# guenthermi/postgres-word2vec

Measured on AMD Instinct MI355X. Metric: batched IVFADC kNN queries/sec (k=5) + recall@5, 3Mx300d, higher is better.
Workload: dtype f32; 1 GPU; IVFADC batch (ivfadc_batch_search generalised to nprobe), 3000000x300d, C=1000, m=12, K=1024, nprobe=10, k=5, batch=1024 queries per GPU, replicated index, queries sharded by rank; N=3000000, d=300, C=1000, m=12, K=1024, nprobe=10, k=5, batch_per_gpu=1024, parallelism=dp1, world_size=1, backend=none (single GPU), batches_in_flight=4

## Files before the change

postgres-word2vec_amd/csrc/fused5.h:

```cpp
#pragma once
#include <hip/hip_runtime.h>
#include <stdint.h>

#include "refine.h"
#include "coarse.h"
#include "scan_tail5.h"

namespace freddy {

static constexpr int SCAN5_G = 16;
static constexpr int SCAN5_PROF_WGS = 1024;

__host__ __device__ __forceinline__ constexpr int filt5_bias(int p, int m) { return FILT5_VMAX + (p < 32768 - FILT5_VMAX * m ? 1 : 0); }
__device__ __forceinline__ uint32_t lane_byte4() {
  uint32_t x;
  asm volatile("v_mbcnt_lo_u32_b32 %0, -1, 0\n\tv_mbcnt_hi_u32_b32 %0, -1, %0\n\tv_lshlrev_b32 %0, 2, %0" : "=v"(x));
  return x;
}
typedef short s2v __attribute__((ext_vector_type(2)));
__device__ __forceinline__ uint32_t pk_add_i16(uint32_t x, uint32_t y) {
  return __builtin_bit_cast(uint32_t, __builtin_bit_cast(s2v, x) + __builtin_bit_cast(s2v, y));
}

template <int S, int QT>
__device__ __forceinline__ void query_codebook5_body(const float* __restrict__ queries, const float* __restrict__ cbT,
                                                     const float* __restrict__ cmax, float* __restrict__ qn,
                                                     float* __restrict__ qscale, uint32_t* __restrict__ qc,
                                                     int Q, int d, int m, int K, int bx, int by, unsigned char* smem,
                                                     uint32_t* __restrict__ qc8 = nullptr) {
  static_assert(QT == 16, "one 16-lane group per query");
  constexpr int SP = (S + 3) & ~3;
  float (*qs)[SP] = reinterpret_cast<float (*)[SP]>(smem);
  float* inv_s = reinterpret_cast<float*>(smem + QT * SP * 4);
  const int tid = threadIdx.x, p = bx, q0 = by * QT;
  static_assert(S <= 32 && SP % 4 == 0, "one k-step of v_mfma_f32_16x16x32_f16 covers a position");
  ch8v bh[8], bl[8];
  auto load_b = [&](int g) {
    const ch8v* src = reinterpret_cast<const ch8v*>(cbT) + ((size_t)p * 8 + g) * (CBF_GROUP_HALVES / 8) + (tid & 63);
#pragma unroll
    for (int t = 0; t < 8; ++t) { bh[t] = src[(size_t)t * 128]; bl[t] = src[(size_t)t * 128 + 64]; }
  };
  load_b((tid >> 6) * 2);
  const int ecb = reinterpret_cast<const int*>(cbT)[cbf_exp_offset(m) + p];
  for (int i = tid; i < QT * SP; i += 256) {
    const int qi = i / SP, j = i - qi * SP;
    qs[qi][j] = (j < S && q0 + qi < Q) ? queries[(size_t)(q0 + qi) * d + p * S + j] : 0.0f;
  }
  {
    const int qi = tid >> 4, pp = tid & 15, q = q0 + qi;
    float best = 0.0f;
    if (pp < m && q < Q) {
      float n2 = 0.0f;
      for (int j = 0; j < S; ++j) { const float v = queries[(size_t)q * d + pp * S + j]; n2 = __builtin_fmaf(v, v, n2); }
      const float nrm = __builtin_sqrtf(n2) * (1.0f + 1e-5f);
      if (p == 0) qn[(size_t)q * m + pp] = nrm;
      best = 2.0f * nrm * cmax[pp];
    }
#pragma unroll
    for (int o = 8; o > 0; o >>= 1) best = fmaxf(best, __shfl_xor(best, o, 64));
    if (pp == 0) {
      const float sc = q < Q ? best * (1.0f / (float)FILT5_VMAX) * (1.0f + 1e-6f) : 0.0f;
      inv_s[qi] = (sc > 0.0f && sc < 1e30f) ? 1.0f / sc : 0.0f;
      if (p == 0 && q < Q) qscale[q] = sc;
    }
  }
  {
    typedef float f4v __attribute__((ext_vector_type(4)));
    __syncthreads();
    const int wave = tid >> 6, lane = tid & 63, col = lane & 15, kq = lane >> 4;
    const int nq = (Q - q0 < QT) ? Q - q0 : QT;
    ch8v ah, al;
    int eq = 0;
    {
      f4v x0 = f4v{0.0f, 0.0f, 0.0f, 0.0f}, x1 = x0;
      if (8 * kq < SP) x0 = *reinterpret_cast<const f4v*>(&qs[col][8 * kq]);
      if (8 * kq + 4 < SP) x1 = *reinterpret_cast<const f4v*>(&qs[col][8 * kq + 4]);
      const float x[8] = {x0.x, x0.y, x0.z, x0.w, x1.x, x1.y, x1.z, x1.w};
      float am = 0.0f;
#pragma unroll
      for (int j = 0; j < 8; ++j) am = fmaxf(am, __builtin_fabsf(x[j]));
      am = fmaxf(am, __shfl_xor(am, 16, 64));
      am = fmaxf(am, __shfl_xor(am, 32, 64));
      if (am > 0.0f && am < 3e38f) { (void)__builtin_frexpf(am, &eq); eq = CBF_EXP - eq; }
#pragma unroll
      for (int j = 0; j < 8; ++j) {
        const float v = __builtin_ldexpf(x[j], eq);
        const _Float16 hh = (_Float16)v;
        ah[j] = hh;
        al[j] = (_Float16)(v - (float)hh);
      }
    }
    int unscale[4];
#pragma unroll
    for (int reg = 0; reg < 4; ++reg) unscale[reg] = -(__shfl(eq, 4 * kq + reg, 64) + ecb);
    const float vmax = (float)FILT5_VMAX;
    const int bias = filt5_bias(p, m);
#pragma unroll
    for (int gg = 0; gg < 2; ++gg) {
      const int g = wave * 2 + gg;
      f4v acc[4][2];
#pragma unroll
      for (int i = 0; i < 4; ++i)
#pragma unroll
        for (int e = 0; e < 2; ++e) acc[i][e] = __builtin_amdgcn_mfma_f32_16x16x32_f16(al, bh[2 * i + e], f4v{0.0f, 0.0f, 0.0f, 0.0f}, 0, 0, 0);
#pragma unroll
      for (int i = 0; i < 4; ++i)
#pragma unroll
        for (int e = 0; e < 2; ++e) acc[i][e] = __builtin_amdgcn_mfma_f32_16x16x32_f16(ah, bl[2 * i + e], acc[i][e], 0, 0, 0);
#pragma unroll
      for (int i = 0; i < 4; ++i)
#pragma unroll
        for (int e = 0; e < 2; ++e) acc[i][e] = __builtin_amdgcn_mfma_f32_16x16x32_f16(ah, bh[2 * i + e], acc[i][e], 0, 0, 0);
      if (gg == 0) load_b(g + 1);
#pragma unroll
      for (int reg = 0; reg < 4; ++reg) {
        const int qi = 4 * kq + reg;
        if (qi < nq) {
          const float inv = inv_s[qi];
          uint32_t wd[4];
#pragma unroll
          for (int i = 0; i < 4; ++i) {
            const int i0 = (int)fminf(fmaxf(__builtin_rintf(-2.0f * __builtin_ldexpf(acc[i][0][reg], unscale[reg]) * inv), -vmax), vmax) + bias;
            const int i1 = (int)fminf(fmaxf(__builtin_rintf(-2.0f * __builtin_ldexpf(acc[i][1][reg], unscale[reg]) * inv), -vmax), vmax) + bias;
            wd[i] = (uint32_t)i0 | ((uint32_t)i1 << 16);
          }
          *reinterpret_cast<uint4*>(qc + ((size_t)(q0 + qi) * m + p) * 512 + 4 * (16 * g + col)) = uint4{wd[0], wd[1], wd[2], wd[3]};
          if (qc8) qc8[((size_t)(q0 + qi) * m + p) * 128 + (16 * g + col)] = (wd[0] & 0xffffu) | (wd[1] << 16);
        }
      }
    }
  }
}
#define FREDDY_TABLE_UNIT_KERNEL __global__ __launch_bounds__(256) __attribute__((amdgpu_waves_per_eu(4)))
template <int S, int QT>
static constexpr int query_codebook5_lds() { return QT * ((S + 3) & ~3) * 4 + QT * 4; }
template <int S, int QT>
FREDDY_TABLE_UNIT_KERNEL void query_codebook5_kernel(const float* __restrict__ queries, const float* __restrict__ cbT,
                                                             const float* __restrict__ cmax, float* __restrict__ qn,
                                                             float* __restrict__ qscale, uint32_t* __restrict__ qc,
                                                             int Q, int d, int m, int K, uint32_t* __restrict__ qc8) {
  __shared__ __attribute__((aligned(16))) unsigned char smem[query_codebook5_lds<S, QT>()];
  query_codebook5_body<S, QT>(queries, cbT, cmax, qn, qscale, qc, Q, d, m, K, blockIdx.x, blockIdx.y, smem, qc8);
}

struct CoarseTableArgs {
  const float* queries;
  const float* coarseF; const float* cn2; float* dist; float* qn2; int Q, Cpad, d, dp; ZeroArgs z; int coarse_gx, coarse_gy;
  const float* cbT; const float* cmax; float* qn; float* qscale; uint32_t* qc; int m, K;
  float* tmin; int C;
  const ch8v* coarseH; int ec;
  uint32_t* qc8;
};
template <int S, int QT, bool H16 = false>
FREDDY_TABLE_UNIT_KERNEL void coarse_table5_kernel(CoarseTableArgs a) {
  extern __shared__ __attribute__((aligned(16))) unsigned char smem[];
  const int n_coarse = a.coarse_gx * a.coarse_gy;
  const int b = blockIdx.x;
  if (b < n_coarse) {
    if constexpr (H16)
      coarse_approx16_body(a.queries, a.coarseH, a.ec, a.cn2, a.dist, a.qn2, a.Q, a.Cpad, a.d, a.z, b % a.coarse_gx, b / a.coarse_gx,
                           a.coarse_gx, a.coarse_gy, smem, a.tmin, a.C);
    else
    coarse_approx_body(a.queries, a.coarseF, a.cn2, a.dist, a.qn2, a.Q, a.Cpad, a.d, a.dp, a.z, b % a.coarse_gx, b / a.coarse_gx,
                       a.coarse_gx, a.coarse_gy, smem, a.tmin, a.C);
  } else {
    const int t = b - n_coarse;
    query_codebook5_body<S, QT>(a.queries, a.cbT, a.cmax, a.qn, a.qscale, a.qc, a.Q, a.d, a.m, a.K, t % a.m, t / a.m, smem, a.qc8);
  }
}

template <int M>
__global__ __launch_bounds__(256) void entry_record5_kernel(RecordArgs a) {
  const int lane = threadIdx.x & 63;
  const int e = blockIdx.x * 4 + (threadIdx.x >> 6);
  if (a.elastic && blockIdx.x == 0 && threadIdx.x == 0) __hip_atomic_fetch_add(a.elastic + EL_PENDING, a.n_announce, FREDDY_RLX_AGENT);
  if (e >= a.n_groups[0]) return;
  const int cell = a.group_cell[e], first = a.group_first[e], gc = a.group_cnt[e];
  const int cnt = gc & 0xff, chunk = gc >> 8;
  int32_t* rec = a.records + (size_t)e * REC_DW;
  if (lane == 0) {
    const int b0 = a.blk_off[cell] + chunk * FUSED_UNIT_BLOCKS;
    int nb = a.blk_off[cell + 1] - b0;
    if (nb > FUSED_UNIT_BLOCKS) nb = FUSED_UNIT_BLOCKS;
    int rows = a.list_off[cell + 1] - a.list_off[cell] - chunk * (FUSED_UNIT_BLOCKS * 64);
    if (rows > FUSED_UNIT_BLOCKS * 64) rows = FUSED_UNIT_BLOCKS * 64;
    rec[0] = cell; rec[1] = cnt; rec[2] = chunk; rec[3] = b0; rec[4] = nb; rec[5] = rows;
  }
  if (lane < 16) {
    const int it = lane < cnt ? a.sorted_item[first + lane] : -1;
    const int q = a.item_query[it >= 0 ? it : a.sorted_item[first]];
    const float sc = a.qscale[q];
    ItemBounds ib = item_bounds(0.0f, 0.0f, a.sentinel);
    if (it >= 0) ib = item_bounds(a.item_dist[it], filter_width5<M>(a.qn + (size_t)q * M, a.pmax, sc), a.sentinel);
    rec[8 + lane] = it;
    rec[24 + lane] = q;
    rec[40 + lane] = (int32_t)__float_as_uint(ib.off);
    rec[56 + lane] = (int32_t)__float_as_uint(ib.e);
    rec[72 + lane] = (int32_t)__float_as_uint(ib.shift);
    rec[88 + lane] = (int32_t)ib.lo_bits;
    rec[104 + lane] = (int32_t)ib.hi_bits;
    rec[128 + lane] = (int32_t)__float_as_uint((it >= 0 && sc < 1e30f) ? sc : 0.0f);
    const float A = it >= 0 ? a.item_dist[it] : -1.0f;
    const bool fin = it >= 0 && ib.e < 1e30f && A >= 0.0f && A < 1e30f;
    rec[144 + lane] = (int32_t)__float_as_uint(fin ? A * (1.0f + 2e-5f) : __uint_as_float(0x7f800000u));
    rec[160 + lane] = (int32_t)__float_as_uint(fin ? A * (1.0f - 2e-5f) : 0.0f);
  }
}

template <int M, bool FULLK, bool CAND, bool PROF, bool U8, bool ELASTIC>
__device__ __forceinline__ void ivf_filter5_body(const FilterArgs& a) {
  static_assert(!(U8 && FULLK), "one byte per code: K <= 256");
  constexpr int G = SCAN5_G, RMAX = FUSED_RMAX, NG = SPEC2_NG;
  constexpr int NP = M / 2;
  constexpr int ROWB = G * 2;
  constexpr int HROWB = 16;
  static_assert(M == 12 && G == 16 && SPEC2_NB == 8, "layout");
  typedef uint32_t u2 __attribute__((ext_vector_type(2)));
  typedef uint32_t u4 __attribute__((ext_vector_type(4)));
  extern __shared__ __attribute__((aligned(16))) unsigned char smem[];
  unsigned char* slab = smem;
  uint32_t* colmin = reinterpret_cast<uint32_t*>(smem + a.desc_offset);
  uint32_t* thr_s = colmin + 16 * 64;
  int32_t* dsc = reinterpret_cast<int32_t*>(smem + a.desc_offset + 4096 + 64);
  int32_t* gidq = dsc + 2 * REC_DW;
  float* rt_s = reinterpret_cast<float*>(gidq + 4);

  const int tid = threadIdx.x, lane = tid & 63;
  const int wave = __builtin_amdgcn_readfirstlane(tid >> 6);
  const bool builder = wave < SPEC2_NB;
  const int K = FULLK ? 1024 : a.K;
  const uint32_t HALFB = (uint32_t)K * HROWB;
  const uint32_t POSB = 2u * HALFB;
  const uint32_t BUFB = 2u * POSB;
  const int n_work = a.n_groups[0];

  int cur = 0, ei = 0;
  const int n_own = ELASTIC ? a.n_own : (int)gridDim.x;
  const bool extra = ELASTIC && (int)blockIdx.x >= n_own;
  if (!extra) {
    if (tid == 0) {
      gidq[0] = (int)blockIdx.x; gidq[1] = n_own + atomicAdd(a.work_counter, 1);
      if constexpr (ELASTIC) {
        __hip_atomic_fetch_sub(a.elastic + EL_PENDING, 1, FREDDY_RLX_AGENT);
        if ((int)blockIdx.x < n_work) __hip_atomic_fetch_add(a.elastic + EL_ACTIVE, 1, FREDDY_RLX_AGENT);
      }
    }
    if (tid < REC_DW) dsc[tid] = a.records[(size_t)blockIdx.x * REC_DW + tid];
  } else if (tid == 0) {
    const int pend = __hip_atomic_load(a.elastic + EL_PENDING, FREDDY_RLX_AGENT);
    const int claims = __hip_atomic_load(a.work_counter, FREDDY_RLX_AGENT);
// ... 341 lines not shown
```

postgres-word2vec_amd/csrc/ivfadc.hip:

```cpp
#include "internal.h"

#include <functional>

#include "kernels.h"
#include "scan_common.h"
#include "fused3.h"
#include "fused5.h"
#include "fused8.h"
#include "one.h"
#include "sparse5.h"
#include "coarse.h"
#include "multi.h"
#include "io_kernels.h"
#include "bigk.h"
#include "ivf_host.h"
#include "query_ids.h"

static void (*scan_kernel(bool m12, int V, bool floor))(ScanArgs) {
  void (*k)(ScanArgs) = nullptr;
  if (floor) return V != 16 ? nullptr : m12 ? &adc_scan_kernel<12, 16, true> : &adc_scan_kernel<0, 16, true>;
  with_V(V, [&](auto v) { k = m12 ? &adc_scan_kernel<12, decltype(v)::value> : &adc_scan_kernel<0, decltype(v)::value>; });
  return k;
}
static void (*filter_kernel(bool whole, bool u8, bool k1024, bool counts_rows, bool prof, bool elastic = false))(FilterArgs) {
// ... 61 lines not shown
  const int passes = (2 * k + BIGK_PASS - 1) / BIGK_PASS;
  const int nsel = passes * BIGK_PASS;
  int npad = 2048;
  while (npad < k + nsel) npad *= 2;
  if (ws->w_bigsel.ensure(sizeof(u64) * (size_t)ma.n_active * nsel) || ws->w_floor.ensure(sizeof(u64) * (size_t)std::max(Q, 1)))
    return fail(FREDDY_E_NOMEM, "workspace allocation failed (k=%d)", k);
  SelectArgs se;
  se.part = sa.part; se.active = ma.active; se.sel = ws->w_bigsel.as<u64>(); se.floor = ws->w_floor.as<u64>();
  se.parts_per_query = ma.parts_per_query; se.nsel = nsel;
  int32_t* const cand_count = sa.cand_count;
  for (int p = 0; p < passes; ++p) {
    sa.floor = p ? ws->w_floor.as<u64>() : nullptr;
    sa.cand_count = p ? nullptr : cand_count;
    if (int rc = launch_scan(ix, s, sa, n_items)) return rc;
    se.pass = p;
    timed_launch(ix, s, "merge_select", [&] { hipLaunchKernelGGL(merge_select_kernel, dim3(ma.n_active), dim3(64), 0, s, se); });
    HIP_TRY(hipGetLastError());
  }
  BigkArgs b;
  b.sel = se.sel; b.active = ma.active; b.pos_to_id = ma.pos_to_id; b.round_rows = ma.round_rows; b.cand_count = ma.cand_count;
  b.out_ids = ma.out_ids; b.out_dist = ma.out_dist; b.found = ma.found; b.next_active = ma.next_active; b.n_next = ma.n_next;
  b.status = ma.status; b.n_active = ma.n_active; b.nsel = nsel; b.npad = npad; b.k = k; b.found_rule = ma.found_rule;
  b.first_round = ma.first_round; b.sentinel = ma.sentinel;
  timed_launch(ix, s, "bigk_replay", [&] {
    hipLaunchKernelGGL(bigk_replay_kernel, dim3(ma.n_active), dim3(BIGK_T), bigk_lds_bytes(npad, k), s, b);
  });
  HIP_TRY(hipGetLastError());
  return 0;
}

int launch_lut(freddy_gpu_index* ix, hipStream_t s, const float* vecs, const int32_t* item_cell,
                      float* lut, int n_items, const float* coarse, const int32_t* item_query) {
  if (n_items <= 0) return 0;
  int ipw = (int)std::max<int64_t>(1, ((int64_t)ix->m * n_items + 4095) / 4096);
  ipw = std::min(ipw, 64);
  dim3 grid((unsigned)ix->m, (unsigned)((n_items + ipw - 1) / ipw));
  const int m = ix->m, K = ix->K, d = ix->d, S = ix->S;
  timed_launch(ix, s, "lut_build", [&] {
    if (S == 25) hipLaunchKernelGGL((lut_build_kernel<25, 4>), grid, dim3(WG), 0, s, vecs, item_cell, ix->cbT, lut, n_items, ipw, m, K, d, coarse, item_query);
    else if (S == 10) hipLaunchKernelGGL((lut_build_kernel<10, 4>), grid, dim3(WG), 0, s, vecs, item_cell, ix->cbT, lut, n_items, ipw, m, K, d, coarse, item_query);
    else if (S == 20) hipLaunchKernelGGL((lut_build_kernel<20, 4>), grid, dim3(WG), 0, s, vecs, item_cell, ix->cbT, lut, n_items, ipw, m, K, d, coarse, item_query);
    else hipLaunchKernelGGL(lut_build_generic_kernel, grid, dim3(WG), 0, s, vecs, item_cell, ix->cbT, lut, n_items, ipw, m, K, d, S, coarse, item_query);
  });
  HIP_TRY(hipGetLastError());
  return 0;
}


static bool ivf_coarse_by_pieces(const IvfRun& r) { return r.approx && r.fused && r.scan_kernel == 5; }
static int ivf_coarse(IvfRun& r, int q_lo = 0, int q_n = -1) {
  Workspace* ws = r.ws;
  freddy_gpu_index* ix = r.ix;
  hipStream_t s = r.s;
  const int Q = r.Q, d = ix->d, C = ix->C, m = ix->m, K = ix->K, Cpad = ix->Cpad;
  if (q_n < 0) { q_lo = 0; q_n = Q; }
  if ((q_lo != 0 || q_n != Q) && !ivf_coarse_by_pieces(r)) return fail(FREDDY_E_ARG, "internal: this path launches its coarse kernel once");
  const int used_words = (C + 31) / 32;
  const bool small_zero = !r.tiled && d <= 1024;
  if (!r.tiled && !small_zero) {
    HIP_TRY(hipMemsetAsync(ws->w_used.p, 0, sizeof(uint32_t) * (size_t)Q * used_words, s));
    HIP_TRY(hipMemsetAsync(ws->w_cnt.p, 0, sizeof(int32_t) * 8, s));
  }
  ZeroArgs za;
  za.p[0] = ws->w_used.as<uint32_t>(); za.n[0] = Q * used_words;
  za.p[1] = ws->w_cnt.as<uint32_t>(); za.n[1] = 8;
  za.p[2] = r.fused ? ws->w_cellcnt.as<uint32_t>() : nullptr; za.n[2] = r.fused ? C * 2 : 0;
  za.p[3] = ws->w_cand.as<uint32_t>(); za.n[3] = 2 * Q;
  za.p[4] = r.fused ? ws->w_surv_cnt.as<uint32_t>() : nullptr; za.n[4] = r.fused ? (int)surv_regions(r, (size_t)Q * r.W) : 0;

  float* tile_min = nullptr;
  if (r.approx && Cpad > COARSE_MAX_CPAD) {
    if (ws->w_tmin.ensure(sizeof(float) * (size_t)Q * (Cpad / 128))) return fail(FREDDY_E_NOMEM, "workspace allocation failed");
    tile_min = ws->w_tmin.as<float>();
  }
  if (ivf_coarse_by_pieces(r)) {
    CoarseTableArgs ct;
    ct.queries = r.d_q + (size_t)q_lo * d; ct.coarseF = ix->coarseP; ct.cn2 = ix->cn2; ct.dist = ws->w_distT.as<float>() + (size_t)q_lo * Cpad;
    ct.qn2 = ws->w_qn2.as<float>() + q_lo;
    ct.Q = q_n; ct.Cpad = Cpad; ct.d = d; ct.dp = ix->dp; ct.z = za; ct.coarse_gx = Cpad / 128; ct.coarse_gy = (q_n + COARSE_TQ - 1) / COARSE_TQ;
    const QueryTable qt = query_table_piece(query_table(ws, ix, Q), ix, q_lo);
    ct.cbT = ix->cbF; ct.cmax = ix->cmaxp; ct.qn = qt.qn; ct.qscale = qt.qscale; ct.qc = qt.qc; ct.qc8 = qt.qc8;
    ct.m = m; ct.K = K; ct.tmin = tile_min ? tile_min + (size_t)q_lo * (Cpad / 128) : nullptr; ct.C = C;
    ct.coarseH = (const ch8v*)ix->coarseH; ct.ec = ix->coarse_ec;
    const size_t lds = std::max<size_t>(ix->coarseH ? coarse_approx16_lds(d) : (size_t)(COARSE_TQ * (ix->dp + 4) + 128) * sizeof(float), (size_t)query_codebook5_lds<25, 16>());
    const unsigned grid = (unsigned)(ct.coarse_gx * ct.coarse_gy + m * ((q_n + 15) / 16));
    timed_launch(ix, s, "coarse_table", [&] {
      if (ix->coarseH) hipLaunchKernelGGL((coarse_table5_kernel<25, 16, true>), dim3(grid), dim3(256), lds, s, ct);
      else hipLaunchKernelGGL((coarse_table5_kernel<25, 16>), dim3(grid), dim3(256), lds, s, ct);
    });
    HIP_TRY(hipGetLastError());
    return 0;
  }
  if (r.fused && r.scan_kernel == 5) {
    const QueryTable qt = query_table(ws, ix, Q);
    timed_launch(ix, s, "query_codebook", [&] {
      hipLaunchKernelGGL((query_codebook5_kernel<25, 16>), dim3(m, (Q + 15) / 16), dim3(256), 0, s, r.d_q, ix->cbF, ix->cmaxp,
                         qt.qn, qt.qscale, qt.qc, Q, d, m, K, qt.qc8);
    });
    HIP_TRY(hipGetLastError());
  }
  timed_launch(ix, s, "coarse_dist", [&] {
    if (r.approx && ix->coarseH)
      hipLaunchKernelGGL(coarse_approx16_kernel, dim3(Cpad / 128, (Q + COARSE_TQ - 1) / COARSE_TQ), dim3(256), coarse_approx16_lds(d), s, r.d_q,
                         (const ch8v*)ix->coarseH, ix->coarse_ec, ix->cn2, ws->w_distT.as<float>(), ws->w_qn2.as<float>(), Q, Cpad, d, za, tile_min, C);
    else if (r.approx)
      hipLaunchKernelGGL(coarse_approx_kernel, dim3(Cpad / 128, (Q + COARSE_TQ - 1) / COARSE_TQ), dim3(256),
                         (size_t)(COARSE_TQ * (ix->dp + 4) + 128) * sizeof(float), s, r.d_q, ix->coarseP, ix->cn2,
                         ws->w_distT.as<float>(), ws->w_qn2.as<float>(), Q, Cpad, d, ix->dp, za, tile_min, C);
    else if (r.tiled)
      hipLaunchKernelGGL((coarse_tile_kernel<2, 16>), dim3(Cpad / 32, (Q + 63) / 64), dim3(256), 0, s, r.d_q, ix->coarseT,
                         ws->w_distT.as<float>(), Q, Cpad, d, za);
    else if (small_zero)
      hipLaunchKernelGGL((coarse_small_kernel<50>), dim3(Cpad / 64, Q), dim3(64), 0, s, r.d_q, ix->coarseT, ws->w_distT.as<float>(), Q, Cpad, d, za);
    else
      hipLaunchKernelGGL((coarse_dist_kernel<16>), dim3(Cpad / WG, (Q + 15) / 16), dim3(WG), (size_t)d * 16 * sizeof(float), s, r.d_q,
                         ix->coarseT, ws->w_distT.as<float>(), Q, Cpad, d);
  });
  HIP_TRY(hipGetLastError());
  return 0;
}

static int ivf_plan(IvfRun& r, PlanArgs& pa) {
  Workspace* ws = r.ws;
  freddy_gpu_index* ix = r.ix;
  hipStream_t s = r.s;
  const int C = ix->C, W = r.W;
  pa = plan_items(r, C);
  pa.dist = ws->w_distT.as<float>(); pa.active = r.active; pa.list_off = ix->list_off;
  pa.used = ws->w_used.as<uint32_t>(); pa.Cpad = ix->Cpad; pa.used_words = (C + 31) / 32;
  pa.cell_count = r.fused ? ws->w_cellcnt.as<int32_t>() : nullptr;
  pa.cell_items = r.fused ? ws->w_sorted.as<int32_t>() : nullptr; pa.cell_cap = r.n_active;
  pa.cell_limit = r.cell_limit;
  const int n_items = r.n_active * W;
  if (r.fused && !(r.zeroed && r.first())) {
    HIP_TRY(hipMemsetAsync(ws->w_cellcnt.p, 0, sizeof(int32_t) * (size_t)C * 2, s));
    HIP_TRY(hipMemsetAsync(ws->w_surv_cnt.p, 0, sizeof(int32_t) * surv_regions(r, (size_t)n_items), s));
  }
  const int PV = pick_V(2 * W);
  const size_t plan_lds = (size_t)(64 + 64 * PV) * sizeof(u64) + (size_t)W * 8;
  if (r.approx) {
    Plan2Args g;
    g.p = pa; g.queries = r.d_q; g.coarse = ix->coarse; g.qn2 = ws->w_qn2.as<float>(); g.item_dist = pa.item_dist;
    g.violations = ix->viol; g.cmax = ix->cmax; g.d = ix->d; g.refine_all = (ix->tune.check_brackets & 2) ? 1 : 0; g.prof = nullptr;
    g.tmin = (r.first() && ix->Cpad > COARSE_MAX_CPAD && ws->w_tmin.p) ? ws->w_tmin.as<float>() : nullptr;
    timed_launch(ix, s, "probe_plan", [&] {
      if (ix->Cpad <= COARSE_MAX_CPAD && r.share > 1) hipLaunchKernelGGL((probe_plan2_kernel<0, false, 1>), dim3(r.n_active), dim3(64), 0, s, g);
      else if (ix->Cpad <= COARSE_MAX_CPAD) hipLaunchKernelGGL((probe_plan2_kernel<0, false>), dim3(r.n_active), dim3(64 * PLAN2_NW), 0, s, g);
      else hipLaunchKernelGGL((probe_plan2_kernel<0, true>), dim3(r.n_active), dim3(64 * PLAN2_NW), 0, s, g);
    });
  } else
  timed_launch(ix, s, "probe_plan", [&] {
    with_V(PV, [&](auto v) { hipLaunchKernelGGL((probe_plan_kernel<decltype(v)::value>), dim3(r.n_active), dim3(64), plan_lds, s, pa); });
  });
  HIP_TRY(hipGetLastError());
  if (!(r.zeroed && r.first())) HIP_TRY(hipMemsetAsync(ws->w_cand.p, 0, sizeof(int32_t) * 2 * r.Q, s));
  return 0;
}

int ivf_work_table(IvfRun& r, WorkTable& wt) {
  Workspace* ws = r.ws;
  freddy_gpu_index* ix = r.ix;
  hipStream_t s = r.s;
  const int n_items = r.n_active * r.W;
  wt = work_counters(ws, ((size_t)n_items / MULTI_G + (size_t)ix->C + 1) * r.upi);
  int32_t* base = ws->w_groups.as<int32_t>();
  wt.group_cell = base; wt.group_first = base + wt.max_groups; wt.group_cnt = base + 2 * wt.max_groups;
  const int sparse_max = r.scan_kernel != 5 ? 0
                         : ix->tune.sparse_items < 0 ? -ix->tune.sparse_items
// ... 673 lines not shown
```

postgres-word2vec_amd/csrc/pq.hip:

```cpp
#include "internal.h"

#include "kernels.h"
#include "scan_common.h"
#include "fused5.h"
#include "one.h"
#include "io_kernels.h"
#include "assign.h"
#include "ivf_host.h"
#include "query_ids.h"

static decltype(&grouping_kernel<0>) grouping_kernel_for(int M2) {
  return M2 == 6 ? &grouping_kernel<6> : M2 == 15 ? &grouping_kernel<15> : &grouping_kernel<0>;
}
static void (*assign_pq_kernel_for(int M2, int RPT))(AssignPqArgs) {
  if (M2 == 6) return RPT == 4 ? &assign_pq_kernel<6, 4> : &assign_pq_kernel<6, 1>;
  return RPT == 4 ? &assign_pq_kernel<0, 4> : &assign_pq_kernel<0, 1>;
}

__global__ __launch_bounds__(256) void pq_shadow_meta_kernel(const int32_t* __restrict__ pos, const int32_t* __restrict__ ids,
                                                            int64_t n_blocks, int64_t n_rows, int lists, int32_t* __restrict__ list_off,
                                                            int32_t* __restrict__ blk_off, int32_t* __restrict__ blk_cell,
                                                            int32_t* __restrict__ pos_ids) {
  const int64_t i = (int64_t)blockIdx.x * 256 + threadIdx.x;
  if (i <= lists) {
// ... 110 lines not shown
  else pq_records_body(a, b - n_table, smem);
}

static int pq_fused_queries_per_chunk(const freddy_gpu_index* ix, int64_t n_blocks) {
  const size_t lists = (size_t)((n_blocks + FUSED_UNIT_BLOCKS - 1) / FUSED_UNIT_BLOCKS);
  size_t n = ((size_t)ix->tune.lut_budget_mb << 20) / (sizeof(u64) * lists * FUSED_NW * FUSED_RMAX * 64);
  n = std::min<size_t>(n, ((size_t)256 << 20) / (sizeof(int32_t) * lists));
  return (int)std::max<size_t>(16, std::min<size_t>(n, 1u << 16));
}

static int pq_view_refresh(freddy_gpu_index* ix, freddy_gpu_index** view, hipStream_t s, const uint32_t* packed, const int32_t* pos,
                           int64_t n_blocks, int64_t n_rows) {
  freddy_gpu_index* fx = *view;
  if (!fx) {
    fx = new freddy_gpu_index();
    fx->shadow_of = ix;
    fx->kind = KIND_IVF; fx->device = ix->device; fx->stream = ix->stream; fx->n_cus = ix->n_cus;
    fx->d = ix->d; fx->m = ix->m; fx->K = ix->K; fx->S = ix->S; fx->M2 = ix->M2;
    if (dev_malloc((void**)&fx->viol, 4 * sizeof(int32_t)) != hipSuccess || hipMemset(fx->viol, 0, 4 * sizeof(int32_t)) != hipSuccess) {
      free_index(fx);
      return fail(FREDDY_E_NOMEM, "device allocation failed (PQ table as pseudo-lists)");
    }
    *view = fx;
  }
  fx->tune = ix->tune;
  fx->cbT = ix->cbT; fx->cbR = ix->cbR; fx->pmax = ix->pmax; fx->cmaxp = ix->cmaxp; fx->cbF = ix->cbF;
  fx->packed = const_cast<uint32_t*>(packed);
  fx->packed8 = (packed == ix->packed) ? ix->packed8 : nullptr; fx->packed8_own = false;
  fx->N = n_rows; fx->n_blocks = n_blocks; fx->max_list_blocks = FUSED_UNIT_BLOCKS;
  const int lists = (int)((n_blocks + FUSED_UNIT_BLOCKS - 1) / FUSED_UNIT_BLOCKS);
  fx->C = lists;
  const size_t slots = (size_t)n_blocks * 64;
  if (fx->v_coarse.ensure(sizeof(float) * (size_t)lists * ix->d) || fx->v_list_off.ensure(sizeof(int32_t) * ((size_t)lists + 1)) ||
      fx->v_blk_off.ensure(sizeof(int32_t) * ((size_t)lists + 1)) || fx->v_blk_cell.ensure(sizeof(int32_t) * (size_t)n_blocks) ||
      fx->v_pos.ensure(sizeof(int32_t) * slots) || fx->v_rterm.ensure(sizeof(float) * slots))
    return fail(FREDDY_E_NOMEM, "device allocation failed (PQ table as pseudo-lists)");
  fx->coarse = fx->v_coarse.as<float>(); fx->list_off = fx->v_list_off.as<int32_t>(); fx->blk_off = fx->v_blk_off.as<int32_t>();
  fx->blk_cell = fx->v_blk_cell.as<int32_t>(); fx->pos = fx->v_pos.as<int32_t>(); fx->rterm = fx->v_rterm.as<float>();
  HIP_TRY(hipMemsetAsync(fx->coarse, 0, sizeof(float) * (size_t)lists * ix->d, s));
  hipLaunchKernelGGL(pq_shadow_meta_kernel, dim3((unsigned)((slots + 255) / 256)), dim3(256), 0, s, pos, ix->ids, n_blocks, n_rows, lists,
                     fx->list_off, fx->blk_off, fx->blk_cell, fx->pos);
  hipLaunchKernelGGL(row_term_kernel, dim3((unsigned)((slots + 255) / 256)), dim3(256), 0, s, fx->packed, fx->blk_cell, fx->coarse, fx->cbR,
                     fx->rterm, (int64_t)slots, fx->M2, fx->d, fx->m, fx->K, fx->S);
  HIP_TRY(hipGetLastError());
  return 0;
}

int pq_shadow_build(freddy_gpu_index* ix) {
  if (ix->pq_shadow) return 0;
  if (int rc = pq_view_refresh(ix, &ix->pq_shadow, ix->stream, ix->packed, ix->pos, ix->n_blocks, ix->N)) {
    if (ix->pq_shadow) { free_index(ix->pq_shadow); ix->pq_shadow = nullptr; }
    return rc;
  }
  HIP_TRY(hipStreamSynchronize(ix->stream));
  return 0;
}


static int pq_fused_chunk(freddy_gpu_index* ix, freddy_gpu_index* fx, hipStream_t s, const float* d_q, int Q, int k, float sentinel,
                          int32_t* d_out_ids, float* d_out_dist) {
  fx->tune = ix->tune;
  Workspace* ws = workspace_for(fx, s);
  const int lists = fx->C, m = fx->m;
  const int SL = (lists >= 32 && Q <= 256 && (size_t)lists * FUSED_NW > 256) ? 4 : 0;
  const int W = SL ? ((lists + SL - 1) / SL) * SL : lists;
  IvfRun r = ivf_run(fx, ws, s, scan_share_now(ix->tune.scan_share, false, ix->device), d_q, Q, k, W, sentinel, d_out_ids, d_out_dist, nullptr);
  r.fused = true; r.records_ready = true; r.merge_slices = SL;
  const size_t n_entries = (size_t)((Q + SCAN5_G - 1) / SCAN5_G) * lists;
  if (ivf_run_ensure(r) || ws->w_records.ensure(sizeof(int32_t) * REC_DW * n_entries))
    return fail(FREDDY_E_NOMEM, "workspace allocation failed (Q=%d over %d pseudo-lists)", Q, lists);
  const PlanArgs pa = plan_items(r, lists);
  const WorkTable wt = work_counters(ws, n_entries);
  const QueryTable qt = query_table(ws, fx, Q);
  PqFrontArgs fa;
  fa.queries = d_q; fa.Q = Q; fa.d = fx->d; fa.lists = lists; fa.W = W; fa.n_rows = fx->N; fa.blk_off = fx->blk_off; fa.list_off = fx->list_off;
  fa.cbT = fx->cbF; fa.cmax = fx->cmaxp; fa.pmax = fx->pmax; fa.qn = qt.qn; fa.qscale = qt.qscale; fa.qc = qt.qc; fa.qc8 = qt.qc8;
  fa.m = m; fa.K = fx->K; fa.sentinel = sentinel; fa.item_cell = pa.item_cell; fa.item_query = pa.item_query;
  fa.item_dist = pa.item_dist; fa.round_rows = pa.round_rows; fa.records = ws->w_records.as<int32_t>(); fa.n_groups = wt.n_groups;
  fa.z.p[0] = ws->w_cnt.as<uint32_t>(); fa.z.n[0] = 1;
  fa.z.p[1] = ws->w_cnt.as<uint32_t>() + 2; fa.z.n[1] = 6;
  fa.z.p[2] = ws->w_cand.as<uint32_t>() + Q; fa.z.n[2] = Q;
  fa.z.p[3] = ws->w_surv_cnt.as<uint32_t>(); fa.z.n[3] = (int)surv_regions(r, (size_t)Q * W);
  fa.z.p[4] = nullptr; fa.z.n[4] = 0;
  const size_t front_lds = std::max<size_t>((size_t)query_codebook5_lds<25, 16>(), (size_t)(1024 + 16 + 2) * sizeof(float));
  timed_launch(fx, s, "pq_front", [&] {
    hipLaunchKernelGGL(pq_front_kernel, dim3((unsigned)(m * ((Q + 15) / 16) + Q)), dim3(256), front_lds, s, fa);
  });
  HIP_TRY(hipGetLastError());
  return ivf_scan_filter(r, pa, wt);
}

static bool pq_one_shape(const freddy_gpu_index* ix, int Q, int k, int64_t n_blocks) {
  return ix->tune.one_launch && !ix->one_launch_failed && Q == 1 && fused_dims(ix) && (ix->K & 3) == 0 && ix->d == 300 &&
         2 * k <= 64 && n_blocks >= 64 && (int64_t)ix->h_ids.size() == ix->N;
}
static int pq_one(freddy_gpu_index* ix, hipStream_t s, const float* h_q, int k, float sentinel, const int32_t* blk_off,
                  const uint32_t* packed, const int32_t* pos, int64_t n_blocks, int32_t* d_out_ids, float* d_out_dist, int32_t* err) {
  Workspace* ws = workspace_for(ix, s);
  const int K = ix->K, L = 2 * k;
  const int G = pq_one_groups(ix->n_cus, L, n_blocks, ONE_WAVES);
  const int chunk_blocks = (int)((n_blocks + G - 1) / G);
  const OneLayout lay{K, 0, 1, L, G};
  uint32_t epoch = 0;
  if (int rc = one_buffer(ws, s, (1ull << 60) | ((uint64_t)K << 32) | ((uint64_t)G << 16) | (uint64_t)L, lay.handoff_bytes(), &epoch)) return rc;
  if (one_prof() && ws->w_one.ensure(256)) return fail(FREDDY_E_NOMEM, "workspace allocation failed");
  OneArgs a;
  memcpy(a.qv, h_q, sizeof(a.qv)); a.cbT = ix->cbT; a.lut_g = ws->w_oneb.as<float>(); a.blk_off = blk_off; a.packed = packed; a.pos = pos;
  a.pos_to_id = nullptr;
  a.part = reinterpret_cast<u64*>(ws->w_oneb.as<char>() + lay.part_off()); a.out_ids = d_out_ids; a.out_dist = d_out_dist;
  a.epoch = epoch; a.err = err;
  a.prof = one_prof() ? ws->w_one.as<unsigned long long>() + 8 : nullptr;
  a.K = K; a.L = L; a.k = k; a.chunk_blocks = chunk_blocks; a.sentinel = sentinel;
  memcpy(&a.sentinel_bits, &sentinel, 4);
  timed_launch(ix, s, "pq_one", [&] { hipLaunchKernelGGL((pq_one_kernel<25>), dim3((unsigned)G), dim3(ONE_WG), lay.lds_bytes(), s, a); });
  HIP_TRY(hipGetLastError());
  ws->one_pending = false;
  return 0;
}

static int pq_queries_per_chunk(const freddy_gpu_index* ix, int64_t n_blocks, int k) {
  const size_t L = (size_t)std::min(2 * k, 1024), nchunk = (size_t)std::max<int64_t>(1, (n_blocks + 63) / 64);
  size_t per_query = sizeof(float) * (size_t)ix->m * ix->K + sizeof(u64) * nchunk * L;
  if (2 * k > 1024) per_query += sizeof(u64) * (size_t)((2 * k + 1024 - 1) / 1024) * 1024;
  const size_t n = ((size_t)ix->tune.lut_budget_mb << 20) / per_query;
  return (int)std::min<size_t>(std::max<size_t>(n, 1), (size_t)1 << 20);
}

static int pq_chunk(freddy_gpu_index* ix, hipStream_t s, const float* d_q, int Q, int k, float sentinel,
                    const int32_t* blk_off, const uint32_t* packed, const int32_t* pos, int64_t n_blocks,
                    int32_t* d_out_ids, float* d_out_dist) {
  Workspace* ws = workspace_for(ix, s);
  const int m = ix->m, K = ix->K;
  const int L = std::min(2 * k, 64 * 16);
  const size_t lutN = (size_t)m * K;
  int chunk_blocks = 64;
  while ((n_blocks + chunk_blocks - 1) / chunk_blocks * (int64_t)Q > 4096 && chunk_blocks < 8192) chunk_blocks *= 2;
  const int nchunk = (int)std::max<int64_t>(1, (n_blocks + chunk_blocks - 1) / chunk_blocks);
  if (ws->w_lut.ensure(sizeof(float) * (size_t)Q * lutN) ||
      ws->w_part.ensure(sizeof(u64) * (size_t)Q * nchunk * L))
    return fail(FREDDY_E_NOMEM, "workspace allocation failed");
  if (int rc = launch_lut(ix, s, d_q, nullptr, ws->w_lut.as<float>(), Q)) return rc;
  ScanArgs sa;
  sa.lut = ws->w_lut.as<float>(); sa.item_list = nullptr; sa.item_query = nullptr;
  sa.blk_off = blk_off; sa.packed = packed; sa.pos = pos; sa.part = ws->w_part.as<u64>();
  sa.cand_count = nullptr;
  sa.m = m; sa.K = K; sa.chunk_blocks = chunk_blocks; sa.nchunk = nchunk; sa.L = L;
  memcpy(&sa.sentinel_bits, &sentinel, 4);
  const MergeArgs ma = merge_args_flat(sa.part, Q, nchunk, L, k, sentinel, ix->ids, d_out_ids, d_out_dist);
  if (2 * k > 1024) return bigk_select_replay(ix, s, ws, sa, Q, ma, Q);
  if (int rc = launch_scan(ix, s, sa, Q)) return rc;
  return launch_merge(ix, s, ma);
}

static int pq_batch(freddy_gpu_index* ix, freddy_gpu_index* view, hipStream_t s, const float* d_q, int Q, int k, float sentinel, const int32_t* blk_off,
                    const uint32_t* packed, const int32_t* pos, int64_t n_blocks, int32_t* d_oi, float* d_od) {
  return for_chunks(Q, view ? pq_fused_queries_per_chunk(ix, n_blocks) : pq_queries_per_chunk(ix, n_blocks, k), [&](int q0, int n) {
    const float* q = d_q + (size_t)q0 * ix->d;
    if (view) return pq_fused_chunk(ix, view, s, q, n, k, sentinel, d_oi + (size_t)q0 * k, d_od + (size_t)q0 * k);
    return pq_chunk(ix, s, q, n, k, sentinel, blk_off, packed, pos, n_blocks, d_oi + (size_t)q0 * k, d_od + (size_t)q0 * k);
  });
}

extern "C" int freddy_gpu_pq_search_dev(freddy_gpu_index_t* ix, const float* d_queries, int32_t Q, int32_t k,
                                        float sentinel, int32_t* d_out_ids, float* d_out_dist, void* hip_stream) {
  if (int rc = check_search_args(ix, KIND_PQ, d_queries, Q, k, d_out_ids, d_out_dist)) return rc;
  if (Q == 0) return FREDDY_OK;
  HIP_TRY(hipSetDevice(ix->device));
// ... 255 lines not shown
```

Measured before the change: 12.67 million queries/s.

## Build query lookup tables for two query groups per block, reusing codebook registers

The query-codebook table part of the fused coarse/table kernel now has each block handle QG (default 2) groups of 16 queries. The codebook fragments held in registers are loaded once and reused across those groups. Query splitting to fp16 hi/lo pairs is staged in LDS, and the next codebook group is prefetched while results are quantised. This halves the number of table blocks and cuts repeated codebook loads, at the cost of more LDS per block, a serial loop over groups within a block, and less block-level parallelism.

```diff
diff --git a/postgres-word2vec_amd/csrc/fused5.h b/postgres-word2vec_amd/csrc/fused5.h
--- a/postgres-word2vec_amd/csrc/fused5.h
+++ b/postgres-word2vec_amd/csrc/fused5.h
@@ -22,13 +22,174 @@
   return __builtin_bit_cast(uint32_t, __builtin_bit_cast(s2v, x) + __builtin_bit_cast(s2v, y));
 }
 
-template <int S, int QT>
+template <int S, int QT, int QG>
+static constexpr int query_codebook5_lds() {
+#if defined(FREDDY_LAB) && defined(FREDDY_LAB_TABLE_FETCH_TWICE)
+  if (QG == 1) return 2048 + 4 * 1024;
+#endif
+  return QG * (QT * ((S + 3) & ~3) * 4 + QT * 4) + (QG > 1 ? QG * (2 * 64 * 16 + QT * 4) : 0);
+}
+
+template <int S, int QT, int QG>
+__device__ __forceinline__ void query_codebook5_groups(const float* __restrict__ queries, const float* __restrict__ cbT,
+                                                       const float* __restrict__ cmax, float* __restrict__ qn,
+                                                       float* __restrict__ qscale, uint32_t* __restrict__ qc,
+                                                       int Q, int d, int m, int bx, int by, unsigned char* smem,
+                                                       uint32_t* __restrict__ qc8) {
+  static_assert(QT == 16 && (QG == 2 || QG == 4), "groups of one 16-lane group per query");
+  static_assert(S <= 32, "one k-step of v_mfma_f32_16x16x32_f16 covers a position");
+  constexpr int SP = (S + 3) & ~3;
+  constexpr int GRP_LDS = QT * SP * 4 + QT * 4;
+  static_assert(GRP_LDS % 16 == 0, "rows, inv_s and the slices behind them stay 16-byte aligned");
+  typedef float f4v __attribute__((ext_vector_type(4)));
+  typedef int i4v __attribute__((ext_vector_type(4)));
+  ch8v* split_s = reinterpret_cast<ch8v*>(smem + QG * GRP_LDS);
+  int* eq_s = reinterpret_cast<int*>(smem + QG * GRP_LDS + QG * 2 * 64 * 16);
+  const int tid = threadIdx.x, lane = tid & 63, col = lane & 15, kq = lane >> 4;
+  const int wave = __builtin_amdgcn_readfirstlane(tid >> 6);
+  const int p = bx, q0 = by * (QT * QG);
+  int n_grp = (Q - q0 + QT - 1) / QT < QG ? (Q - q0 + QT - 1) / QT : QG;
+  asm volatile("" : "+s"(n_grp));
+  ch8v bh[8], bl[8];
+  auto load_b_half = [&](int g, int h) {
+    const char* src = reinterpret_cast<const char*>(cbT) + ((size_t)p * 8 + g) * (CBF_GROUP_HALVES * 2);
+    const uint32_t l16 = lane_byte4() * 4u;
+#pragma unroll
+    for (int t = 4 * h; t < 4 * h + 4; ++t) {
+      bh[t] = *reinterpret_cast<const ch8v*>(src + t * 2048 + l16);
+      bl[t] = *reinterpret_cast<const ch8v*>(src + t * 2048 + 1024 + l16);
+    }
+  };
+  load_b_half(wave * 2, 0);
+  load_b_half(wave * 2, 1);
+  const int ecb = reinterpret_cast<const int*>(cbT)[cbf_exp_offset(m) + p];
+#pragma unroll 1
+  for (int grp = 0; grp < n_grp; ++grp) {
+    float (*qs)[SP] = reinterpret_cast<float (*)[SP]>(smem + grp * GRP_LDS);
+    float* inv_s = reinterpret_cast<float*>(smem + grp * GRP_LDS + QT * SP * 4);
+    const int qg0 = q0 + grp * QT;
+    for (int i = tid; i < QT * SP; i += 256) {
+      const int qi = i / SP, j = i - qi * SP;
+      qs[qi][j] = (j < S && qg0 + qi < Q) ? queries[(size_t)(qg0 + qi) * d + p * S + j] : 0.0f;
+    }
+    const int qi = tid >> 4, pp = tid & 15, q = qg0 + qi;
+    float best = 0.0f;
+    if (pp < m && q < Q) {
+      float n2 = 0.0f;
+      for (int j = 0; j < S; ++j) { const float v = queries[(size_t)q * d + pp * S + j]; n2 = __builtin_fmaf(v, v, n2); }
+      const float nrm = __builtin_sqrtf(n2) * (1.0f + 1e-5f);
+      if (p == 0) qn[(size_t)q * m + pp] = nrm;
+      best = 2.0f * nrm * cmax[pp];
+    }
+#pragma unroll
+    for (int o = 8; o > 0; o >>= 1) best = fmaxf(best, __shfl_xor(best, o, 64));
+    if (pp == 0) {
+      const float sc = q < Q ? best * (1.0f / (float)FILT5_VMAX) * (1.0f + 1e-6f) : 0.0f;
+      inv_s[qi] = (sc > 0.0f && sc < 1e30f) ? 1.0f / sc : 0.0f;
+      if (p == 0 && q < Q) qscale[q] = sc;
+    }
+  }
+  __syncthreads();
+  for (int grp = wave; grp < n_grp; grp += 4) {
+    const float (*qs)[SP] = reinterpret_cast<const float (*)[SP]>(smem + grp * GRP_LDS);
+    f4v x0 = f4v{0.0f, 0.0f, 0.0f, 0.0f}, x1 = x0;
+    if (8 * kq < SP) x0 = *reinterpret_cast<const f4v*>(&qs[col][8 * kq]);
+    if (8 * kq + 4 < SP) x1 = *reinterpret_cast<const f4v*>(&qs[col][8 * kq + 4]);
+    const float x[8] = {x0.x, x0.y, x0.z, x0.w, x1.x, x1.y, x1.z, x1.w};
+    float am = 0.0f;
+#pragma unroll
+    for (int j = 0; j < 8; ++j) am = fmaxf(am, __builtin_fabsf(x[j]));
+    am = fmaxf(am, __shfl_xor(am, 16, 64));
+    am = fmaxf(am, __shfl_xor(am, 32, 64));
+    int eq = 0;
+    if (am > 0.0f && am < 3e38f) { (void)__builtin_frexpf(am, &eq); eq = CBF_EXP - eq; }
+    ch8v ah, al;
+#pragma unroll
+    for (int j = 0; j < 8; ++j) {
+      const float v = __builtin_ldexpf(x[j], eq);
+      const _Float16 hh = (_Float16)v;
+      ah[j] = hh;
+      al[j] = (_Float16)(v - (float)hh);
+    }
+    split_s[(grp * 2 + 0) * 64 + lane] = ah;
+    split_s[(grp * 2 + 1) * 64 + lane] = al;
+    if (kq == 0) eq_s[grp * QT + col] = eq;
+  }
+  __syncthreads();
+  const float vmax = (float)FILT5_VMAX;
+  const int bias = filt5_bias(p, m);
+  const uint32_t lane_row = (uint32_t)(4 * kq * m) * 2048u + (uint32_t)col * 16u;
+  const uint32_t lane_row8 = (uint32_t)(4 * kq * m) * 512u + (uint32_t)col * 4u;
+  auto pass = [&](int grp, int g, auto next) {
+    constexpr int next_g_off = decltype(next)::value;
+    const int qg0 = q0 + grp * QT;
+    const int nq = (Q - qg0 < QT) ? Q - qg0 : QT;
+    const ch8v ah = split_s[(grp * 2 + 0) * 64 + lane], al = split_s[(grp * 2 + 1) * 64 + lane];
+    const i4v eq4 = *reinterpret_cast<const i4v*>(eq_s + grp * QT + 4 * kq);
+    const f4v inv4 = *reinterpret_cast<const f4v*>(smem + grp * GRP_LDS + QT * SP * 4 + 16 * kq);
+    uint32_t wd[4][4];
+#pragma unroll
+    for (int h = 0; h < 2; ++h) {
+      f4v acc[2][2];
+#pragma unroll
+      for (int i = 0; i < 2; ++i)
+#pragma unroll
+        for (int e = 0; e < 2; ++e) acc[i][e] = __builtin_amdgcn_mfma_f32_16x16x32_f16(al, bh[4 * h + 2 * i + e], f4v{0.0f, 0.0f, 0.0f, 0.0f}, 0, 0, 0);
+#pragma unroll
+      for (int i = 0; i < 2; ++i)
+#pragma unroll
+        for (int e = 0; e < 2; ++e) acc[i][e] = __builtin_amdgcn_mfma_f32_16x16x32_f16(ah, bl[4 * h + 2 * i + e], acc[i][e], 0, 0, 0);
+#pragma unroll
+      for (int i = 0; i < 2; ++i)
+#pragma unroll
+        for (int e = 0; e < 2; ++e) acc[i][e] = __builtin_amdgcn_mfma_f32_16x16x32_f16(ah, bh[4 * h + 2 * i + e], acc[i][e], 0, 0, 0);
+      if constexpr (next_g_off != 0) load_b_half(g + next_g_off, h);
+      __builtin_amdgcn_sched_barrier(0);
+#pragma unroll
+      for (int reg = 0; reg < 4; ++reg) {
+        const int unscale = -(eq4[reg] + ecb);
+        const float inv = inv4[reg];
+#pragma unroll
+        for (int i = 0; i < 2; ++i) {
+          const int i0 = (int)fminf(fmaxf(__builtin_rintf(-2.0f * __builtin_ldexpf(acc[i][0][reg], unscale) * inv), -vmax), vmax) + bias;
+          const int i1 = (int)fminf(fmaxf(__builtin_rintf(-2.0f * __builtin_ldexpf(acc[i][1][reg], unscale) * inv), -vmax), vmax) + bias;
+          wd[reg][2 * h + i] = (uint32_t)i0 | ((uint32_t)i1 << 16);
+          asm volatile("" : "+v"(wd[reg][2 * h + i]));
+        }
+      }
+      __builtin_amdgcn_sched_barrier(0);
+    }
+    char* row = reinterpret_cast<char*>(qc) + ((size_t)qg0 * m + p) * 2048 + g * 256;
+    char* row8 = reinterpret_cast<char*>(qc8) + ((size_t)qg0 * m + p) * 512 + g * 64;
+#pragma unroll
+    for (int reg = 0; reg < 4; ++reg) {
+      if (4 * kq + reg < nq) {
+        *reinterpret_cast<uint4*>(row + (size_t)reg * m * 2048 + lane_row) = uint4{wd[reg][0], wd[reg][1], wd[reg][2], wd[reg][3]};
+        if (qc8) *reinterpret_cast<uint32_t*>(row8 + (size_t)reg * m * 512 + lane_row8) = (wd[reg][0] & 0xffffu) | (wd[reg][1] << 16);
+      }
+    }
+  };
+#pragma unroll
+  for (int gg = 0; gg < 2; ++gg) {
+    const int g = wave * 2 + gg;
+#pragma unroll 1
+    for (int grp = 0; grp < n_grp - 1; ++grp) pass(grp, g, std::integral_constant<int, 0>{});
+    if (gg == 0) pass(n_grp - 1, g, std::integral_constant<int, 1>{});
+    else pass(n_grp - 1, g, std::integral_constant<int, 0>{});
+  }
+}
+
+template <int S, int QT, int QG = 1>
 __device__ __forceinline__ void query_codebook5_body(const float* __restrict__ queries, const float* __restrict__ cbT,
                                                      const float* __restrict__ cmax, float* __restrict__ qn,
                                                      float* __restrict__ qscale, uint32_t* __restrict__ qc,
                                                      int Q, int d, int m, int K, int bx, int by, unsigned char* smem,
                                                      uint32_t* __restrict__ qc8 = nullptr) {
   static_assert(QT == 16, "one 16-lane group per query");
+  if constexpr (QG > 1) {
+    query_codebook5_groups<S, QT, QG>(queries, cbT, cmax, qn, qscale, qc, Q, d, m, bx, by, smem, qc8);
+    return;
+  }
   constexpr int SP = (S + 3) & ~3;
   float (*qs)[SP] = reinterpret_cast<float (*)[SP]>(smem);
   float* inv_s = reinterpret_cast<float*>(smem + QT * SP * 4);
@@ -39,6 +200,13 @@
     const ch8v* src = reinterpret_cast<const ch8v*>(cbT) + ((size_t)p * 8 + g) * (CBF_GROUP_HALVES / 8) + (tid & 63);
 #pragma unroll
     for (int t = 0; t < 8; ++t) { bh[t] = src[(size_t)t * 128]; bl[t] = src[(size_t)t * 128 + 64]; }
+#if defined(FREDDY_LAB) && defined(FREDDY_LAB_TABLE_FETCH_TWICE)
+    const ch8v* dup = reinterpret_cast<const ch8v*>(cbT) + ((size_t)((p + 1) % m) * 8 + g) * (CBF_GROUP_HALVES / 8) + (tid & 63);
+#pragma unroll
+    for (int t = 0; t < 16; ++t)
+      __builtin_amdgcn_global_load_lds((const __attribute__((address_space(1))) void*)(dup + (size_t)t * 64),
+                                       (__attribute__((address_space(3))) void*)(smem + 2048 + (tid >> 6) * 1024), 16, 0, 0);
+#endif
   };
   load_b((tid >> 6) * 2);
   const int ecb = reinterpret_cast<const int*>(cbT)[cbf_exp_offset(m) + p];
@@ -133,16 +301,18 @@
 }
 #define FREDDY_TABLE_UNIT_KERNEL __global__ __launch_bounds__(256) __attribute__((amdgpu_waves_per_eu(4)))
 template <int S, int QT>
-static constexpr int query_codebook5_lds() { return QT * ((S + 3) & ~3) * 4 + QT * 4; }
-template <int S, int QT>
 FREDDY_TABLE_UNIT_KERNEL void query_codebook5_kernel(const float* __restrict__ queries, const float* __restrict__ cbT,
                                                              const float* __restrict__ cmax, float* __restrict__ qn,
                                                              float* __restrict__ qscale, uint32_t* __restrict__ qc,
                                                              int Q, int d, int m, int K, uint32_t* __restrict__ qc8) {
-  __shared__ __attribute__((aligned(16))) unsigned char smem[query_codebook5_lds<S, QT>()];
+  __shared__ __attribute__((aligned(16))) unsigned char smem[query_codebook5_lds<S, QT, 1>()];
   query_codebook5_body<S, QT>(queries, cbT, cmax, qn, qscale, qc, Q, d, m, K, blockIdx.x, blockIdx.y, smem, qc8);
 }
 
+#ifndef FREDDY_COARSE_TABLE_QG
+#define FREDDY_COARSE_TABLE_QG 2
+#endif
+static constexpr int COARSE_TABLE_QG = FREDDY_COARSE_TABLE_QG;
 struct CoarseTableArgs {
   const float* queries;
   const float* coarseF; const float* cn2; float* dist; float* qn2; int Q, Cpad, d, dp; ZeroArgs z; int coarse_gx, coarse_gy;
@@ -165,7 +335,7 @@
                        a.coarse_gx, a.coarse_gy, smem, a.tmin, a.C);
   } else {
     const int t = b - n_coarse;
-    query_codebook5_body<S, QT>(a.queries, a.cbT, a.cmax, a.qn, a.qscale, a.qc, a.Q, a.d, a.m, a.K, t % a.m, t / a.m, smem, a.qc8);
+    query_codebook5_body<S, QT, COARSE_TABLE_QG>(a.queries, a.cbT, a.cmax, a.qn, a.qscale, a.qc, a.Q, a.d, a.m, a.K, t % a.m, t / a.m, smem, a.qc8);
   }
 }
 
diff --git a/postgres-word2vec_amd/csrc/ivfadc.hip b/postgres-word2vec_amd/csrc/ivfadc.hip
--- a/postgres-word2vec_amd/csrc/ivfadc.hip
+++ b/postgres-word2vec_amd/csrc/ivfadc.hip
@@ -167,8 +167,8 @@
     ct.cbT = ix->cbF; ct.cmax = ix->cmaxp; ct.qn = qt.qn; ct.qscale = qt.qscale; ct.qc = qt.qc; ct.qc8 = qt.qc8;
     ct.m = m; ct.K = K; ct.tmin = tile_min ? tile_min + (size_t)q_lo * (Cpad / 128) : nullptr; ct.C = C;
     ct.coarseH = (const ch8v*)ix->coarseH; ct.ec = ix->coarse_ec;
-    const size_t lds = std::max<size_t>(ix->coarseH ? coarse_approx16_lds(d) : (size_t)(COARSE_TQ * (ix->dp + 4) + 128) * sizeof(float), (size_t)query_codebook5_lds<25, 16>());
-    const unsigned grid = (unsigned)(ct.coarse_gx * ct.coarse_gy + m * ((q_n + 15) / 16));
+    const size_t lds = std::max<size_t>(ix->coarseH ? coarse_approx16_lds(d) : (size_t)(COARSE_TQ * (ix->dp + 4) + 128) * sizeof(float), (size_t)query_codebook5_lds<25, 16, COARSE_TABLE_QG>());
+    const unsigned grid = (unsigned)(ct.coarse_gx * ct.coarse_gy + m * ((q_n + 16 * COARSE_TABLE_QG - 1) / (16 * COARSE_TABLE_QG)));
     timed_launch(ix, s, "coarse_table", [&] {
       if (ix->coarseH) hipLaunchKernelGGL((coarse_table5_kernel<25, 16, true>), dim3(grid), dim3(256), lds, s, ct);
       else hipLaunchKernelGGL((coarse_table5_kernel<25, 16>), dim3(grid), dim3(256), lds, s, ct);
diff --git a/postgres-word2vec_amd/csrc/pq.hip b/postgres-word2vec_amd/csrc/pq.hip
--- a/postgres-word2vec_amd/csrc/pq.hip
+++ b/postgres-word2vec_amd/csrc/pq.hip
@@ -216,7 +216,7 @@
   fa.z.p[2] = ws->w_cand.as<uint32_t>() + Q; fa.z.n[2] = Q;
   fa.z.p[3] = ws->w_surv_cnt.as<uint32_t>(); fa.z.n[3] = (int)surv_regions(r, (size_t)Q * W);
   fa.z.p[4] = nullptr; fa.z.n[4] = 0;
-  const size_t front_lds = std::max<size_t>((size_t)query_codebook5_lds<25, 16>(), (size_t)(1024 + 16 + 2) * sizeof(float));
+  const size_t front_lds = std::max<size_t>((size_t)query_codebook5_lds<25, 16, 1>(), (size_t)(1024 + 16 + 2) * sizeof(float));
   timed_launch(fx, s, "pq_front", [&] {
     hipLaunchKernelGGL(pq_front_kernel, dim3((unsigned)(m * ((Q + 15) / 16) + Q)), dim3(256), front_lds, s, fa);
   });
```

Result: no change. 12.67 million queries/s (-0.1%).
